# Z-yq/TensorflowASR

Hardware: AMD Instinct MI355X
Metric: audio-frames/sec/GPU + RTF, ConformerCTC(S) 10s utts, 1/2/4/8 MI355X (higher is better)
Workload: dtype f32

## Files before the change

tensorflowasr_amd/csrc/attention_split.hip:

```cpp
#include <cstdlib>

#include "common.h"
#include "env.h"
#include "launch.h"
#include "mfma_ops.h"

MI355_SCALAR_F32_BEGIN

namespace {

#ifndef MI355ASR_ATTN_DIAG
#define MI355ASR_ATTN_DIAG 0
#endif
constexpr int ADG = MI355ASR_ATTN_DIAG;
constexpr int HS = 36;
constexpr int TPK = 256;
constexpr int NKT = TPK / 16;
constexpr int NST = TPK / 32;
constexpr int OT = 3;
constexpr int AW = 16;
constexpr int ATH = AW * 64;

template <int TM>
__global__ __launch_bounds__(ATH) void attention_split_kernel(AttnArgs a) {
  static_assert(TM == 3 || ADG == 0, "the timing variants are those of the three-term kernel");
  __shared__ __attribute__((aligned(16))) u32x4_t Kf[TM][NKT][64];
  __shared__ __attribute__((aligned(16))) float Kt[NKT][64];
  __shared__ __attribute__((aligned(16))) u32x4_t Vf[TM][NST][OT][64];
  const float sq = TM == 2 ? a.h2_sq : 1.f, sk = TM == 2 ? a.h2_sk : 1.f, sv = TM == 2 ? a.h2_sv : 1.f;
  constexpr float SP = TM == 2 ? 16384.f : 1.f;

  const int tid = threadIdx.x, lane = tid & 63, wv = tid >> 6;
  const int g = lane >> 4, g4 = g * 4, c = lane & 15;
  const int TS = a.Tk, TQ = a.Tq;
  const int h = blockIdx.y, b = blockIdx.z;
  const int T = a.k_len ? min(a.k_len[b], TS) : TS;
  const int ld = a.ldk, D = a.D;
  const size_t khead = a.head_major ? ((size_t)b * a.H + h) * TS * HS : (size_t)b * TS * ld + h * HS;
  const float* __restrict__ kbase = a.k + khead;
  const float* __restrict__ vbase = a.v + khead;

  const int qt = blockIdx.x * AW + wv;
  const int tq = qt * 16 + c;
  const float* qrow = a.head_major ? a.q + (((size_t)b * a.H + h) * TQ + min(tq, TQ - 1)) * HS
                                   : a.q + ((size_t)b * TQ + min(tq, TQ - 1)) * a.ldq + h * HS;
  constexpr float LOG2E = 1.4426950408889634f;
  const f32x4 qlo = ldg4(qrow + 8 * g), qhi = ldg4(qrow + 8 * g + 4);
  const float qtl = qrow[32 + g] * (LOG2E * sq);

  const int skey = 16 * wv + c;
  const float* krow = kbase + (size_t)min(skey, T - 1) * ld;
  f32x4 klo = ldg4(krow + 8 * g), khi = ldg4(krow + 8 * g + 4);
  float ktl = krow[32 + g];
  constexpr int NVE = NST * OT * 64, NVT = (NVE + ATH - 1) / ATH;
  float ve[NVT][8];
#pragma unroll
  for (int it = 0; it < NVT; ++it) {
    const int en = tid + it * ATH;
    const int s = en / (OT * 64), rem = en - s * (OT * 64), ot = rem >> 6, l = rem & 63, kg = l >> 4, fc = l & 15;
    const int f = 16 * ot + fc;
#pragma unroll
    for (int j = 0; j < 8; ++j) {
      const int key = 32 * s + 16 * (j >> 2) + 4 * kg + (j & 3);
      ve[it][j] = (!(ADG & 16) && en < NVE && f < HS && key < T) ? vbase[(size_t)key * ld + f] : 0.f;
    }
  }
  if (skey >= T) { klo = splat4(0.f); khi = splat4(0.f); ktl = 0.f; }
  {
    const Split8x3 kf = split_tm<TM>(klo * splat4(sk), khi * splat4(sk));
    Kf[0][wv][lane] = kf.t[0];
    Kf[1][wv][lane] = kf.t[1];
    if constexpr (TM == 3) Kf[2][wv][lane] = kf.t[2];
    Kt[wv][lane] = ktl * sk;
  }
  __syncthreads();
  const bool active = qt * 16 < TQ;
  const int nkt = (T + 15) / 16;
  const Split8x3 qf = split_tm<TM>(qlo * splat4(LOG2E * sq), qhi * splat4(LOG2E * sq));
  const f32x4 inv_qk = splat4(1.0f / (sq * sk));

  f32x4 sc[NKT];
  auto qk_tile = [&](int kt) {
    const u32x4_t kf[3] = {Kf[0][kt][lane], Kf[1][kt][lane], Kf[TM - 1][kt][lane]};
    const float kl = Kt[kt][lane];
    if constexpr (ADG & 1) { sc[kt] = splat4(kl) + __builtin_bit_cast(f32x4, kf[0]); return; }
    f32x4 acc = mma_tm<TM>(kf, qf, splat4(0.f));
    sc[kt] = mfma4(kl, qtl, acc);
    if constexpr (TM == 2) sc[kt] = sc[kt] * inv_qk;
  };
  const bool full = (nkt == NKT);
  if (active) {
    if (full) {
#pragma unroll
      for (int kt = 0; kt < NKT; ++kt) qk_tile(kt);
    } else {
#pragma unroll
      for (int kt = 0; kt < NKT; ++kt) {
        if (kt < nkt) qk_tile(kt); else sc[kt] = splat4(-INFINITY);
      }
    }
  }

#pragma unroll
  for (int it = 0; it < NVT; ++it) {
    const int en = tid + it * ATH;
    if (en < NVE && !(ADG & 8)) {
      const f32x4 lo = {ve[it][0], ve[it][1], ve[it][2], ve[it][3]}, hi = {ve[it][4], ve[it][5], ve[it][6], ve[it][7]};
      const Split8x3 vf = split_tm<TM>(lo * splat4(sv), hi * splat4(sv));
      u32x4_t* dst = &Vf[0][0][0][0] + en;
      dst[0] = vf.t[0];
      dst[NVE] = vf.t[1];
      if constexpr (TM == 3) dst[2 * NVE] = vf.t[2];
    }
  }
  if (!active) { __syncthreads(); return; }

  float mx = -INFINITY;
#pragma unroll
  for (int kt = 0; kt < NKT; ++kt) {
    if (kt < nkt && 16 * kt + 16 > T) {
      const int kb = 16 * kt + g4;
      sc[kt].x = (kb + 0 < T) ? sc[kt].x : -INFINITY;
      sc[kt].y = (kb + 1 < T) ? sc[kt].y : -INFINITY;
      sc[kt].z = (kb + 2 < T) ? sc[kt].z : -INFINITY;
      sc[kt].w = (kb + 3 < T) ? sc[kt].w : -INFINITY;
    }
    mx = fmaxf(mx, fmaxf(fmaxf(sc[kt].x, sc[kt].y), fmaxf(sc[kt].z, sc[kt].w)));
  }
  mx = group_max(mx);
  float psum = 0.f;
#pragma unroll
  for (int kt = 0; kt < NKT; ++kt) {
    if constexpr (!(ADG & 2)) {
      sc[kt].x = __builtin_amdgcn_exp2f(sc[kt].x - mx);
      sc[kt].y = __builtin_amdgcn_exp2f(sc[kt].y - mx);
      sc[kt].z = __builtin_amdgcn_exp2f(sc[kt].z - mx);
      sc[kt].w = __builtin_amdgcn_exp2f(sc[kt].w - mx);
    }
    psum += (sc[kt].x + sc[kt].y) + (sc[kt].z + sc[kt].w);
  }

  __syncthreads();
  f32x4 o[OT];
#pragma unroll
  for (int i = 0; i < OT; ++i) o[i] = splat4(0.f);
  const int nst = (nkt + 1) / 2;
#pragma unroll
  for (int s = 0; s < NST; ++s) {
    if constexpr (ADG & 4) { o[0] += sc[2 * s]; o[1] += sc[2 * s + 1]; }
    else if (s < nst) {
      const Split8x3 pf = split_tm<TM>(sc[2 * s] * splat4(SP), sc[2 * s + 1] * splat4(SP));
#pragma unroll
      for (int i = 0; i < OT; ++i) {
        const u32x4_t vf[3] = {Vf[0][s][i][lane], Vf[1][s][i][lane], Vf[TM - 1][s][i][lane]};
        o[i] = mma_tm<TM>(vf, pf, o[i]);
      }
    }
  }
  const float inv = (1.0f / group_sum(psum)) * (1.0f / (SP * sv));
  if (tq < TQ) {
    float* orow = a.ctx + ((size_t)b * TQ + tq) * D + h * HS;
#pragma unroll
    for (int i = 0; i < OT; ++i) {
      if (16 * i + g4 < HS) stg4(orow + 16 * i + g4, o[i] * splat4(inv));
    }
  }
}


constexpr int LKB = 256;
constexpr int LKT = LKB / 16;
constexpr int LST = LKB / 32;
template <int TM, int LW>
__global__ __launch_bounds__(LW * 64) void attention_split_long_kernel(AttnArgs a) {
  constexpr int LTH = LW * 64;
  constexpr bool LPRE = LW <= 8;
  __shared__ __attribute__((aligned(16))) u32x4_t Kf[TM][LKT][64];
  __shared__ __attribute__((aligned(16))) float Kt[LKT][64];
  __shared__ __attribute__((aligned(16))) u32x4_t Vf[TM][LST][OT][64];
  const float sq = TM == 2 ? a.h2_sq : 1.f, sk = TM == 2 ? a.h2_sk : 1.f, sv = TM == 2 ? a.h2_sv : 1.f;
  constexpr float SP = TM == 2 ? 16384.f : 1.f;
  const int tid = threadIdx.x, lane = tid & 63, wv = tid >> 6;
  const int g = lane >> 4, g4 = g * 4, c = lane & 15;
  const int TS = a.Tk, TQ = a.Tq;
  const int h = blockIdx.y, b = blockIdx.z;
  const int T = a.k_len ? min(a.k_len[b], TS) : TS;
  const int ld = a.ldk, D = a.D;
  const size_t khead = a.head_major ? ((size_t)b * a.H + h) * TS * HS : (size_t)b * TS * ld + h * HS;
  const float* __restrict__ kbase = a.k + khead;
  const float* __restrict__ vbase = a.v + khead;
  const int qt = blockIdx.x * LW + wv;
  const int tq = qt * 16 + c;
  const float* qrow = a.head_major ? a.q + (((size_t)b * a.H + h) * TQ + min(tq, TQ - 1)) * HS
                                   : a.q + ((size_t)b * TQ + min(tq, TQ - 1)) * a.ldq + h * HS;
  constexpr float LOG2E = 1.4426950408889634f;
  const f32x4 qlo = ldg4(qrow + 8 * g), qhi = ldg4(qrow + 8 * g + 4);
  const float qtl = qrow[32 + g] * (LOG2E * sq);
  const Split8x3 qf = split_tm<TM>(qlo * splat4(LOG2E * sq), qhi * splat4(LOG2E * sq));
  const f32x4 inv_qk = splat4(1.0f / (sq * sk));
  const bool active = qt * 16 < TQ;

  constexpr int NKE = LKT * 64, NKR = (NKE + LTH - 1) / LTH;
  constexpr int NVE = LST * OT * 64, NVR = (NVE + LTH - 1) / LTH;
  f32x4 klo[NKR], khi[NKR];
  float ktl[NKR];
  float ve[NVR][8];
  const unsigned uld = (unsigned)ld;
  auto fetch = [&](int kb0) {
#pragma unroll
    for (int it = 0; it < NKR; ++it) {
      const int en = tid + it * LTH, kt = en >> 6, l = en & 63, kg = l >> 4, kc = l & 15;
      const int skey = kb0 + 16 * kt + kc;
      const unsigned ko = (unsigned)min(skey, T - 1) * uld + 8u * kg;
      const bool ok = en < NKE && skey < T;
      klo[it] = ok ? *reinterpret_cast<const f32x4*>(kbase + ko) : splat4(0.f);
      khi[it] = ok ? *reinterpret_cast<const f32x4*>(kbase + ko + 4u) : splat4(0.f);
      ktl[it] = ok ? kbase[(unsigned)min(skey, T - 1) * uld + 32u + kg] : 0.f;
    }
#pragma unroll
    for (int it = 0; it < NVR; ++it) {
      const int en = tid + it * LTH;
      const int s = en / (OT * 64), rem = en - s * (OT * 64), ot = rem >> 6, l = rem & 63, kg = l >> 4, fc = l & 15;
      const int f = 16 * ot + fc;
      const int key0 = kb0 + 32 * s + 4 * kg;
      const unsigned vo = (unsigned)key0 * uld + (unsigned)f;
#pragma unroll
      for (int j = 0; j < 8; ++j) {
        const int dk = 16 * (j >> 2) + (j & 3);
        ve[it][j] = (en < NVE && f < HS && key0 + dk < T) ? vbase[vo + (unsigned)dk * uld] : 0.f;
      }
    }
  };
  auto stage = [&]() {
#pragma unroll
    for (int it = 0; it < NKR; ++it) {
      const int en = tid + it * LTH;
      if (en < NKE) {
        const Split8x3 kf = split_tm<TM>(klo[it] * splat4(sk), khi[it] * splat4(sk));
        (&Kf[0][0][0])[en] = kf.t[0];
        (&Kf[1][0][0])[en] = kf.t[1];
        if constexpr (TM == 3) (&Kf[2][0][0])[en] = kf.t[2];
        (&Kt[0][0])[en] = ktl[it] * sk;
      }
    }
#pragma unroll
    for (int it = 0; it < NVR; ++it) {
      const int en = tid + it * LTH;
      if (en < NVE) {
        const f32x4 lo = {ve[it][0], ve[it][1], ve[it][2], ve[it][3]}, hi = {ve[it][4], ve[it][5], ve[it][6], ve[it][7]};
        const Split8x3 vf = split_tm<TM>(lo * splat4(sv), hi * splat4(sv));
        u32x4_t* dst = &Vf[0][0][0][0] + en;
        dst[0] = vf.t[0];
        dst[NVE] = vf.t[1];
        if constexpr (TM == 3) dst[2 * NVE] = vf.t[2];
      }
    }
  };

  float m = -INFINITY, psum = 0.f;
  f32x4 o[OT];
#pragma unroll
  for (int i = 0; i < OT; ++i) o[i] = splat4(0.f);
  if constexpr (LPRE) fetch(0);
#pragma unroll 1
  for (int kb0 = 0; kb0 < T; kb0 += LKB) {
    if constexpr (!LPRE) fetch(kb0);
    stage();
    __syncthreads();
    if constexpr (LPRE) {
      if (kb0 + LKB < T) fetch(kb0 + LKB);
    }
    if (active) {
      const int nk = min(T - kb0, LKB), nkt = (nk + 15) / 16;
      constexpr int NH = LPRE ? 2 : 4, HT = LKT / NH, HS2 = LST / NH;
#pragma unroll
      for (int hb = 0; hb < NH; ++hb) {
        if (hb * HT < nkt) {
          f32x4 sc[HT];
#pragma unroll
          for (int k8 = 0; k8 < HT; ++k8) {
            const int kt = hb * HT + k8;
            if (kt < nkt) {
              const u32x4_t kf[3] = {Kf[0][kt][lane], Kf[1][kt][lane], Kf[TM - 1][kt][lane]};
              f32x4 acc = mma_tm<TM>(kf, qf, splat4(0.f));
              sc[k8] = mfma4(Kt[kt][lane], qtl, acc);
              if constexpr (TM == 2) sc[k8] = sc[k8] * inv_qk;
            } else {
              sc[k8] = splat4(-INFINITY);
            }
          }
          float bm = -INFINITY;
#pragma unroll
          for (int k8 = 0; k8 < HT; ++k8) {
            const int kt = hb * HT + k8;
            if (kt < nkt && 16 * kt + 16 > nk) {
              const int kk = 16 * kt + g4;
              sc[k8].x = (kk + 0 < nk) ? sc[k8].x : -INFINITY;
              sc[k8].y = (kk + 1 < nk) ? sc[k8].y : -INFINITY;
              sc[k8].z = (kk + 2 < nk) ? sc[k8].z : -INFINITY;
              sc[k8].w = (kk + 3 < nk) ? sc[k8].w : -INFINITY;
            }
            bm = fmaxf(bm, fmaxf(fmaxf(sc[k8].x, sc[k8].y), fmaxf(sc[k8].z, sc[k8].w)));
          }
          const float mn = fmaxf(m, group_max(bm));
          const float alpha = __builtin_amdgcn_exp2f(m - mn);
          m = mn;
          float bs = 0.f;
#pragma unroll
          for (int k8 = 0; k8 < HT; ++k8) {
            sc[k8].x = __builtin_amdgcn_exp2f(sc[k8].x - mn);
            sc[k8].y = __builtin_amdgcn_exp2f(sc[k8].y - mn);
            sc[k8].z = __builtin_amdgcn_exp2f(sc[k8].z - mn);
            sc[k8].w = __builtin_amdgcn_exp2f(sc[k8].w - mn);
            bs += (sc[k8].x + sc[k8].y) + (sc[k8].z + sc[k8].w);
          }
          psum = psum * alpha + bs;
#pragma unroll
          for (int i = 0; i < OT; ++i) o[i] = o[i] * splat4(alpha);
          const int nst = (nkt + 1) / 2;
#pragma unroll
          for (int s4 = 0; s4 < HS2; ++s4) {
            const int s = hb * HS2 + s4;
            if (s < nst) {
              const Split8x3 pf = split_tm<TM>(sc[2 * s4] * splat4(SP), sc[2 * s4 + 1] * splat4(SP));
#pragma unroll
              for (int i = 0; i < OT; ++i) {
                const u32x4_t vf[3] = {Vf[0][s][i][lane], Vf[1][s][i][lane], Vf[TM - 1][s][i][lane]};
                o[i] = mma_tm<TM>(vf, pf, o[i]);
              }
            }
          }
        }
      }
    }
    __syncthreads();
  }
  if (!active) return;
  const float inv = (1.0f / group_sum(psum)) * (1.0f / (SP * sv));
  if (tq < TQ) {
    float* orow = a.ctx + ((size_t)b * TQ + tq) * D + h * HS;
#pragma unroll
    for (int i = 0; i < OT; ++i) {
      if (16 * i + g4 < HS) stg4(orow + 16 * i + g4, o[i] * splat4(inv));
    }
  }
}

}

bool attention_split_applicable(int hs, const AttnArgs& a) {
  static_assert(TPK == ATTN_SPLIT_SHORT_KEYS, "launch.h names the key count of the one-block kernel");
  return hs == HS && a.win_front < 0 && a.Tk > 16 && a.Tq > 16 && a.ldk % 4 == 0 && a.ldq % 4 == 0;
}
bool attention_split_two_term_fits(const AttnArgs& a) { return a.h2_sq > 0.f && a.h2_sk > 0.f && a.h2_sv > 0.f && ADG == 0; }

int launch_attention_split(int hs, const AttnArgs& a, int terms, hipStream_t s) {
  if (!attention_split_applicable(hs, a) || (terms != 2 && terms != 3) || (terms == 2 && !attention_split_two_term_fits(a))) return -1;
  const int qtiles = (a.Tq + 15) / 16;
  const bool two = terms == 2;
  if (a.head_major && (!two || a.ldq != HS || a.ldk != HS)) return -1;
  note_scheme(two ? SCHEME_F16X2 : SCHEME_BF16X3);
  const dim3 grid((qtiles + AW - 1) / AW, a.H, a.B);
  if (a.Tk > TPK) {
    static const int ncu = [] { hipDeviceProp_t p; int d = 0; return (hipGetDevice(&d) == hipSuccess && hipGetDeviceProperties(&p, d) == hipSuccess) ? p.multiProcessorCount : 256; }();
    const long n16 = (long)((qtiles + 15) / 16) * a.H * a.B, n8 = (long)((qtiles + 7) / 8) * a.H * a.B;
    const double c16 = (double)((n16 + ncu - 1) / ncu), c8 = 0.62 * (double)((n8 + ncu - 1) / ncu);
    if (c16 <= c8) {
      const dim3 gl((qtiles + 15) / 16, a.H, a.B);
      if (two) hipLaunchKernelGGL((attention_split_long_kernel<2, 16>), gl, dim3(1024), 0, s, a);
      else hipLaunchKernelGGL((attention_split_long_kernel<3, 16>), gl, dim3(1024), 0, s, a);
    } else {
      const dim3 gl((qtiles + 7) / 8, a.H, a.B);
      if (two) hipLaunchKernelGGL((attention_split_long_kernel<2, 8>), gl, dim3(512), 0, s, a);
      else hipLaunchKernelGGL((attention_split_long_kernel<3, 8>), gl, dim3(512), 0, s, a);
    }
    return 0;
  }
  if (two)
    hipLaunchKernelGGL(attention_split_kernel<2>, grid, dim3(ATH), 0, s, a);
  else
    hipLaunchKernelGGL(attention_split_kernel<3>, grid, dim3(ATH), 0, s, a);
  return 0;
}

MI355_SCALAR_F32_END
```

Measured before the change: 35.74 million.

## Load K/V through buffer resources and fold QK rescale into exp2 argument

Replaces the clamped global loads of K and V rows in both attention kernels with raw buffer loads. Out-of-range keys land past the descriptor's extent and return zero in hardware, which removes the per-element bounds selects and min clamps. Separately, the two-term variant no longer multiplies every score tile by 1/(sq*sk); the scaling is folded into an fma inside the exp2 argument, with the running max kept in unscaled units. A new applicability guard keeps buffer offsets within 31 bits, which could route some large shapes away from this kernel.

```diff
diff --git a/tensorflowasr_amd/csrc/attention_split.hip b/tensorflowasr_amd/csrc/attention_split.hip
--- a/tensorflowasr_amd/csrc/attention_split.hip
+++ b/tensorflowasr_amd/csrc/attention_split.hip
@@ -21,6 +21,37 @@
 constexpr int AW = 16;
 constexpr int ATH = AW * 64;
 
+DEV __amdgpu_buffer_rsrc_t head_rows_rsrc(const float* base, int T, int ld) {
+  return __builtin_amdgcn_make_buffer_rsrc((void*)base, 0, T > 0 ? ((T - 1) * ld + HS) * 4 : 0, 0x00020000);
+}
+DEV float buf_ld(__amdgpu_buffer_rsrc_t r, unsigned byte_off) {
+  return __builtin_bit_cast(float, __builtin_amdgcn_raw_buffer_load_b32(r, (int)byte_off, 0, 0));
+}
+DEV f32x4 buf_ld4(__amdgpu_buffer_rsrc_t r, unsigned byte_off) {
+  return __builtin_bit_cast(f32x4, __builtin_amdgcn_raw_buffer_load_b128(r, (int)byte_off, 0, 0));
+}
+constexpr unsigned BUF_OUT = 0x80000000u;
+
+DEV void load_k_entry(__amdgpu_buffer_rsrc_t krs, bool in, int key, int kg, unsigned ld, f32x4& klo, f32x4& khi, float& ktl) {
+  const unsigned ko = in ? (unsigned)key * ld * 4u + 32u * kg : BUF_OUT;
+  klo = buf_ld4(krs, ko);
+  khi = buf_ld4(krs, ko + 16u);
+  ktl = buf_ld(krs, ko + 128u - 28u * kg);
+}
+DEV void gather_v_entry(__amdgpu_buffer_rsrc_t vrs, int en, int entries, int kb0, unsigned ld, float (&ve)[8]) {
+  const int s = en / (OT * 64), rem = en - s * (OT * 64), ot = rem >> 6, l = rem & 63, kg = l >> 4, fc = l & 15;
+  const int f = 16 * ot + fc;
+  const unsigned rowb = ld * 4u;
+  const unsigned vo = (en < entries && f < HS) ? (unsigned)(kb0 + 32 * s + 4 * kg) * rowb + 4u * f : BUF_OUT;
+#pragma unroll
+  for (int j = 0; j < 8; ++j) ve[j] = buf_ld(vrs, vo + (unsigned)(16 * (j >> 2) + (j & 3)) * rowb);
+}
+
+template <int TM>
+DEV float scaled_diff(float x, float s, float nms) {
+  if constexpr (TM == 2) return __builtin_fmaf(x, s, nms); else return x + nms;
+}
+
 template <int TM>
 __global__ __launch_bounds__(ATH) void attention_split_kernel(AttnArgs a) {
   static_assert(TM == 3 || ADG == 0, "the timing variants are those of the three-term kernel");
@@ -48,24 +79,14 @@
   const f32x4 qlo = ldg4(qrow + 8 * g), qhi = ldg4(qrow + 8 * g + 4);
   const float qtl = qrow[32 + g] * (LOG2E * sq);
 
-  const int skey = 16 * wv + c;
-  const float* krow = kbase + (size_t)min(skey, T - 1) * ld;
-  f32x4 klo = ldg4(krow + 8 * g), khi = ldg4(krow + 8 * g + 4);
-  float ktl = krow[32 + g];
+  f32x4 klo, khi;
+  float ktl;
+  load_k_entry(head_rows_rsrc(kbase, T, ld), true, 16 * wv + c, g, (unsigned)ld, klo, khi, ktl);
   constexpr int NVE = NST * OT * 64, NVT = (NVE + ATH - 1) / ATH;
   float ve[NVT][8];
-#pragma unroll
-  for (int it = 0; it < NVT; ++it) {
-    const int en = tid + it * ATH;
-    const int s = en / (OT * 64), rem = en - s * (OT * 64), ot = rem >> 6, l = rem & 63, kg = l >> 4, fc = l & 15;
-    const int f = 16 * ot + fc;
-#pragma unroll
-    for (int j = 0; j < 8; ++j) {
-      const int key = 32 * s + 16 * (j >> 2) + 4 * kg + (j & 3);
-      ve[it][j] = (!(ADG & 16) && en < NVE && f < HS && key < T) ? vbase[(size_t)key * ld + f] : 0.f;
-    }
-  }
-  if (skey >= T) { klo = splat4(0.f); khi = splat4(0.f); ktl = 0.f; }
+  const __amdgpu_buffer_rsrc_t vrs = head_rows_rsrc(vbase, T, ld);
+#pragma unroll
+  for (int it = 0; it < NVT; ++it) gather_v_entry(vrs, tid + it * ATH, (ADG & 16) ? 0 : NVE, 0, (unsigned)ld, ve[it]);
   {
     const Split8x3 kf = split_tm<TM>(klo * splat4(sk), khi * splat4(sk));
     Kf[0][wv][lane] = kf.t[0];
@@ -77,7 +98,7 @@
   const bool active = qt * 16 < TQ;
   const int nkt = (T + 15) / 16;
   const Split8x3 qf = split_tm<TM>(qlo * splat4(LOG2E * sq), qhi * splat4(LOG2E * sq));
-  const f32x4 inv_qk = splat4(1.0f / (sq * sk));
+  const float inv_qk = 1.0f / (sq * sk);
 
   f32x4 sc[NKT];
   auto qk_tile = [&](int kt) {
@@ -86,7 +107,6 @@
     if constexpr (ADG & 1) { sc[kt] = splat4(kl) + __builtin_bit_cast(f32x4, kf[0]); return; }
     f32x4 acc = mma_tm<TM>(kf, qf, splat4(0.f));
     sc[kt] = mfma4(kl, qtl, acc);
-    if constexpr (TM == 2) sc[kt] = sc[kt] * inv_qk;
   };
   const bool full = (nkt == NKT);
   if (active) {
@@ -129,13 +149,14 @@
   }
   mx = group_max(mx);
   float psum = 0.f;
+  const float nmx = -(mx * inv_qk);
 #pragma unroll
   for (int kt = 0; kt < NKT; ++kt) {
     if constexpr (!(ADG & 2)) {
-      sc[kt].x = __builtin_amdgcn_exp2f(sc[kt].x - mx);
-      sc[kt].y = __builtin_amdgcn_exp2f(sc[kt].y - mx);
-      sc[kt].z = __builtin_amdgcn_exp2f(sc[kt].z - mx);
-      sc[kt].w = __builtin_amdgcn_exp2f(sc[kt].w - mx);
+      sc[kt].x = __builtin_amdgcn_exp2f(scaled_diff<TM>(sc[kt].x, inv_qk, nmx));
+      sc[kt].y = __builtin_amdgcn_exp2f(scaled_diff<TM>(sc[kt].y, inv_qk, nmx));
+      sc[kt].z = __builtin_amdgcn_exp2f(scaled_diff<TM>(sc[kt].z, inv_qk, nmx));
+      sc[kt].w = __builtin_amdgcn_exp2f(scaled_diff<TM>(sc[kt].w, inv_qk, nmx));
     }
     psum += (sc[kt].x + sc[kt].y) + (sc[kt].z + sc[kt].w);
   }
@@ -197,7 +218,7 @@
   const f32x4 qlo = ldg4(qrow + 8 * g), qhi = ldg4(qrow + 8 * g + 4);
   const float qtl = qrow[32 + g] * (LOG2E * sq);
   const Split8x3 qf = split_tm<TM>(qlo * splat4(LOG2E * sq), qhi * splat4(LOG2E * sq));
-  const f32x4 inv_qk = splat4(1.0f / (sq * sk));
+  const float inv_qk = 1.0f / (sq * sk);
   const bool active = qt * 16 < TQ;
 
   constexpr int NKE = LKT * 64, NKR = (NKE + LTH - 1) / LTH;
@@ -206,30 +227,15 @@
   float ktl[NKR];
   float ve[NVR][8];
   const unsigned uld = (unsigned)ld;
+  const __amdgpu_buffer_rsrc_t krs = head_rows_rsrc(kbase, T, ld), vrs = head_rows_rsrc(vbase, T, ld);
   auto fetch = [&](int kb0) {
 #pragma unroll
     for (int it = 0; it < NKR; ++it) {
-      const int en = tid + it * LTH, kt = en >> 6, l = en & 63, kg = l >> 4, kc = l & 15;
-      const int skey = kb0 + 16 * kt + kc;
-      const unsigned ko = (unsigned)min(skey, T - 1) * uld + 8u * kg;
-      const bool ok = en < NKE && skey < T;
-      klo[it] = ok ? *reinterpret_cast<const f32x4*>(kbase + ko) : splat4(0.f);
-      khi[it] = ok ? *reinterpret_cast<const f32x4*>(kbase + ko + 4u) : splat4(0.f);
-      ktl[it] = ok ? kbase[(unsigned)min(skey, T - 1) * uld + 32u + kg] : 0.f;
-    }
-#pragma unroll
-    for (int it = 0; it < NVR; ++it) {
-      const int en = tid + it * LTH;
-      const int s = en / (OT * 64), rem = en - s * (OT * 64), ot = rem >> 6, l = rem & 63, kg = l >> 4, fc = l & 15;
-      const int f = 16 * ot + fc;
-      const int key0 = kb0 + 32 * s + 4 * kg;
-      const unsigned vo = (unsigned)key0 * uld + (unsigned)f;
-#pragma unroll
-      for (int j = 0; j < 8; ++j) {
-        const int dk = 16 * (j >> 2) + (j & 3);
-        ve[it][j] = (en < NVE && f < HS && key0 + dk < T) ? vbase[vo + (unsigned)dk * uld] : 0.f;
-      }
-    }
+      const int en = tid + it * LTH, kt = en >> 6, l = en & 63;
+      load_k_entry(krs, en < NKE, kb0 + 16 * kt + (l & 15), l >> 4, uld, klo[it], khi[it], ktl[it]);
+    }
+#pragma unroll
+    for (int it = 0; it < NVR; ++it) gather_v_entry(vrs, tid + it * LTH, NVE, kb0, uld, ve[it]);
   };
   auto stage = [&]() {
 #pragma unroll
@@ -284,7 +290,6 @@
               const u32x4_t kf[3] = {Kf[0][kt][lane], Kf[1][kt][lane], Kf[TM - 1][kt][lane]};
               f32x4 acc = mma_tm<TM>(kf, qf, splat4(0.f));
               sc[k8] = mfma4(Kt[kt][lane], qtl, acc);
-              if constexpr (TM == 2) sc[k8] = sc[k8] * inv_qk;
             } else {
               sc[k8] = splat4(-INFINITY);
             }
@@ -303,15 +308,16 @@
             bm = fmaxf(bm, fmaxf(fmaxf(sc[k8].x, sc[k8].y), fmaxf(sc[k8].z, sc[k8].w)));
           }
           const float mn = fmaxf(m, group_max(bm));
-          const float alpha = __builtin_amdgcn_exp2f(m - mn);
+          const float nmn = -(mn * inv_qk);
+          const float alpha = __builtin_amdgcn_exp2f(scaled_diff<TM>(m, inv_qk, nmn));
           m = mn;
           float bs = 0.f;
 #pragma unroll
           for (int k8 = 0; k8 < HT; ++k8) {
-            sc[k8].x = __builtin_amdgcn_exp2f(sc[k8].x - mn);
-            sc[k8].y = __builtin_amdgcn_exp2f(sc[k8].y - mn);
-            sc[k8].z = __builtin_amdgcn_exp2f(sc[k8].z - mn);
-            sc[k8].w = __builtin_amdgcn_exp2f(sc[k8].w - mn);
+            sc[k8].x = __builtin_amdgcn_exp2f(scaled_diff<TM>(sc[k8].x, inv_qk, nmn));
+            sc[k8].y = __builtin_amdgcn_exp2f(scaled_diff<TM>(sc[k8].y, inv_qk, nmn));
+            sc[k8].z = __builtin_amdgcn_exp2f(scaled_diff<TM>(sc[k8].z, inv_qk, nmn));
+            sc[k8].w = __builtin_amdgcn_exp2f(scaled_diff<TM>(sc[k8].w, inv_qk, nmn));
             bs += (sc[k8].x + sc[k8].y) + (sc[k8].z + sc[k8].w);
           }
           psum = psum * alpha + bs;
@@ -350,7 +356,7 @@
 
 bool attention_split_applicable(int hs, const AttnArgs& a) {
   static_assert(TPK == ATTN_SPLIT_SHORT_KEYS, "launch.h names the key count of the one-block kernel");
-  return hs == HS && a.win_front < 0 && a.Tk > 16 && a.Tq > 16 && a.ldk % 4 == 0 && a.ldq % 4 == 0;
+  return hs == HS && a.win_front < 0 && a.Tk > 16 && a.Tq > 16 && a.ldk % 4 == 0 && a.ldq % 4 == 0 && (long long)a.Tk * a.ldk * 4 < (1LL << 31);
 }
 bool attention_split_two_term_fits(const AttnArgs& a) { return a.h2_sq > 0.f && a.h2_sk > 0.f && a.h2_sv > 0.f && ADG == 0; }
 
```

Measured after the change: 36.01 million, median of 5. Within noise of the previous version (+0.8%).
